# ThatRedox/ChunkyClPlugin

Hardware: AMD Instinct MI355X
Metric: Msamples/s, 32x32-chunk scene @1920x1080 (higher is better)
Workload: dtype f32

## Files before the change

### __graft_entry__.py

```python
import os
import sys

ROOT = os.path.dirname(os.path.abspath(__file__))
if ROOT not in sys.path:
    sys.path.insert(0, ROOT)


def build() -> None:
    from chunkyclplugin_amd import native
    path = native.build()
    native.build_tuning()
    lib = native.lib()
    missing = [s for s in native.declared_symbols() if not hasattr(lib, s)]
    if missing:
        raise RuntimeError(f"{path} does not export {missing}")
    from oracle import binding
    binding.port()
    binding.ref()
    binding.port_libm()
    binding.ref_libm()
    import subprocess
    out = os.path.join(native.CSRC, "build", "ubench_gather.o")
    os.makedirs(os.path.dirname(out), exist_ok=True)
    proc = subprocess.run(["hipcc", "--offload-arch=gfx950", "-O3", "-c", os.path.join(ROOT, "tools", "ubench_gather.hip"), "-o", out],
                          capture_output=True, text=True)
    if proc.returncode != 0:
        raise RuntimeError("hipcc failed on tools/ubench_gather.hip:\n" + proc.stderr[-2000:])
    exe = os.path.join(native.CSRC, "build", "host_example")
    proc = subprocess.run(["g++", "-std=c++17", "-I" + os.path.join(ROOT, "include"), os.path.join(ROOT, "examples", "host_example.cpp"), "-o", exe,
                           "-L" + native.PKG_DIR, "-lchunky_hip", "-Wl,-rpath," + native.PKG_DIR, "-Wl,--allow-shlib-undefined"],
                          capture_output=True, text=True)
    if proc.returncode != 0:
        raise RuntimeError("g++ failed on examples/host_example.cpp:\n" + proc.stderr[-2000:])
    import chunkyclplugin_amd


def smoke() -> None:
    import numpy as np
    from chunkyclplugin_amd import scenes
    from chunkyclplugin_amd.renderer import HipPathTracingRenderer, HipSceneLoader, RendererInstance
    from oracle import binding

    sc = scenes.tiny_scene(width=96, height=64)
    seeds = scenes.java_random_ints(4)
    inst = RendererInstance.get(0)
    loader = HipSceneLoader(inst)
    loader.load_packed(sc)
    r = HipPathTracingRenderer(loader, sc.width, sc.height)
    r.set_camera(sc.projector_type, sc.camera)
    r.render_passes(seeds)
# ... 17 lines not shown
```

### chunkyclplugin_amd/csrc/capi_host.cpp

```cpp
#include "capi_host.hpp"

#include <cmath>
#include <cstring>
#include <mutex>

#include "../../include/chunky_hip.h"
#include "camera_proj.h"
#include "capi_error.hpp"
#include "rt_math.h"
#include "widetree.hpp"

using namespace chunky;

int check_ints(const int32_t* p, int64_t n, const char* what) {
    if (n < 0 || (n > 0 && !p)) return fail(CHUNKY_E_INVALID, "%s: bad array (n=%lld)", what, (long long)n);
    return CHUNKY_OK;
}

static_assert(RT_PROJ_PARALLEL == CHUNKY_PROJ_PARALLEL && RT_PROJ_FISHEYE == CHUNKY_PROJ_FISHEYE && RT_PROJ_PANORAMIC == CHUNKY_PROJ_PANORAMIC &&
                  RT_PROJ_PANORAMIC_SLOT == CHUNKY_PROJ_PANORAMIC_SLOT && RT_PROJ_STEREOGRAPHIC == CHUNKY_PROJ_STEREOGRAPHIC &&
                  RT_PROJ_ODS == CHUNKY_PROJ_ODS && RT_PROJ_ODS_STACKED == CHUNKY_PROJ_ODS_STACKED, "camera_proj.h");
bool is_projected_type(int type) {
    return (type >= CHUNKY_PROJ_PARALLEL && type <= CHUNKY_PROJ_STEREOGRAPHIC) || type == CHUNKY_PROJ_ODS || type == CHUNKY_PROJ_ODS_STACKED;
}
int check_projected(const char* who, int type, const float* s, int64_t n, int height) {
    if (!is_projected_type(type))
        return fail(CHUNKY_E_INVALID, "%s: projector type %d is not a projected camera (1-5, 7, 8)", who, type);
    if (!s) return fail(CHUNKY_E_INVALID, "%s: NULL settings", who);
    if (n != 15) return fail(CHUNKY_E_INVALID, "%s: projector type %d needs 15 floats, got %lld", who, type, (long long)n);
    for (int i = 0; i < 15; i++)
        if (!std::isfinite(s[i])) return fail(CHUNKY_E_INVALID, "%s: settings[%d] is not finite", who, i);
    if (s[12] != 0.0f) return fail(CHUNKY_E_INVALID, "%s: settings[12] must be 0 for projector type %d (its lens is set by chunky_render_set_lens)", who, type);
    if (!(s[14] > 0.0f)) return fail(CHUNKY_E_INVALID, "%s: settings[14] must be > 0, got %g", who, (double)s[14]);
    if (s[13] != 0.0f && (type == CHUNKY_PROJ_FISHEYE || type == CHUNKY_PROJ_PANORAMIC || type == CHUNKY_PROJ_STEREOGRAPHIC))
        return fail(CHUNKY_E_INVALID, "%s: settings[13] must be 0 for projector type %d", who, type);
    if (type == CHUNKY_PROJ_ODS_STACKED) {
        if (s[13] < 0.0f) return fail(CHUNKY_E_INVALID, "%s: the stacked ODS image needs an eye offset >= 0, got %g", who, (double)s[13]);
        if (height % 2 != 0) return fail(CHUNKY_E_INVALID, "%s: the stacked ODS image needs an even height, got %d", who, height);
// ... 102 lines not shown
```

### chunkyclplugin_amd/csrc/capi_scene.hip

```cpp
#include "capi_internal.hpp"

#ifndef CHUNKY_BVH_TOP_RECORDS
#define CHUNKY_BVH_TOP_RECORDS 0
#endif
#ifndef CHUNKY_BVH_TREELET_RECORDS
#define CHUNKY_BVH_TREELET_RECORDS 0
#endif
static void bvh_layout_params(int* top, int* treelet) {
    *top = CHUNKY_BVH_TOP_RECORDS;
    *treelet = CHUNKY_BVH_TREELET_RECORDS;
#ifdef CHUNKY_TUNING
    if (const char* e = getenv("CHUNKY_BVH_LAYOUT")) {
        int a = 0, b = 0;
        if (sscanf(e, "%d,%d", &a, &b) == 2 && a >= 0 && b >= 0) {
            *top = a;
            *treelet = b;
        }
    }
#endif
}

extern "C" int chunky_scene_create(chunky_ctx* ctx, chunky_scene** out) {
    if (!ctx || !out) return fail(CHUNKY_E_INVALID, "chunky_scene_create: NULL argument");
    std::unique_ptr<chunky_scene> s(new chunky_scene);
// ... 306 lines not shown
            s->tri_off = nodes.size() * 4;
            nodes.insert(nodes.end(), tris.begin(), tris.end());
            HIP_TRY(s->bvh_rec.upload(nodes.data(), nodes.size() * 4, s->ctx->stream));
        }
        s->bvh_dirty = false;
    }
    if (want_emitters)
        if (int rc = refresh_emitters(s)) return rc;
    v->emitters = want_emitters ? (const int4*)s->emitters.p : nullptr;
    v->n_emitters = want_emitters ? (int)(s->host_emitters.size() / 4) : 0;
    v->n_block_ints = (int)(s->host_blocks.size() < 0x7FFFFFFFu ? s->host_blocks.size() : 0x7FFFFFFFu);
    v->sort_blocks = s->model_leaf_permille >= kSortBlocksPermille ? 1 : 0;
    v->bvh_rec = (const int4*)s->bvh_rec.p;
    v->tri_rec = s->bvh_rec.p ? (const int4*)((const char*)s->bvh_rec.p + s->tri_off) : nullptr;
    v->tri_off = (unsigned)s->tri_off;
    v->world_root = s->world_root;
    v->actor_root = s->actor_root;
    v->quad_aux = (const float*)s->quad_aux.p;
    v->bvh_stack_entries = (s->world_height > s->actor_height ? s->world_height : s->actor_height) + 1;
    v->block_info = (const int4*)s->block_info.p;
    v->mat8 = (const int4*)s->mat8.p;
    v->aabb_rec = (const int4*)s->aabb_rec.p;
    v->quad_rec = (const int4*)s->quad_rec.p;
    v->wide = s->wide_meta.nlev > 0 ? (const uint32_t*)s->wide.p : nullptr;
    v->wide_nlev = s->wide_meta.nlev;
    for (int i = 0; i < 6; i++) {
        v->wide_shift[i] = s->wide_meta.shift[i];
        v->wide_bits[i] = s->wide_meta.bits[i];
    }
    return CHUNKY_OK;
}
```

### chunkyclplugin_amd/csrc/path_state.hpp

```cpp
#pragma once
#include <hip/hip_runtime.h>

#include "kernels.hpp"
#include "rt_device.hpp"

namespace chunky {

struct LdsStack {
    int* base;
    int stride;
    DEV void push(int slot, int v) { base[slot * stride] = v; }
    DEV int pop(int slot) { return base[slot * stride]; }
};
template <int TREE>
DEV void leaf_lookup(const SceneView& S, int bx, int by, int bz, int& data, int& level, int& kind, bool inside = true, int* entry = nullptr) {
    if (TREE < 16 && !inside) bx = by = bz = 0;
    if (TREE == 0) {
        const int* __restrict__ tree = S.octree;
        level = S.octree_depth;
        data = tree[0];
        while (data > 0) {
            level--;
            data = tree[data + ((((bx >> level) & 1) << 2) | (((by >> level) & 1) << 1) | ((bz >> level) & 1))];
        }
        data = -data;
        kind = (data == 0 || data == kAnyType || (unsigned)data + 1u >= (unsigned)S.n_block_ints) ? 2 : 1;
    } else {
        const uint32_t* __restrict__ tree = S.wide;
        int e = 0;
        if (TREE >= 16) {
            constexpr int N3 = TREE - 16;
            {
                const int tb = S.wide_bits[0];
                unsigned idx = (((((unsigned)bx >> (3 * N3)) << tb) | ((unsigned)by >> (3 * N3))) << tb) | ((unsigned)bz >> (3 * N3));
                idx = inside ? idx : 0u;
                e = *(const int*)((const char*)tree + (idx << 2));
            }
#pragma unroll
            for (int i = 0; i < N3; i++) {
                if (e >= 0) {
                    const int sh = 3 * (N3 - 1 - i);
                    const unsigned xs = sh <= 6 ? (unsigned)bx << (6 - sh) : (unsigned)bx >> (sh - 6);
                    const unsigned ys = sh <= 3 ? (unsigned)by << (3 - sh) : (unsigned)by >> (sh - 3);
                    unsigned idx = ((unsigned)bz >> sh) & 7u;
                    asm("v_and_or_b32 %0, %1, 56, %0" : "+v"(idx) : "v"(ys));
                    asm("v_and_or_b32 %0, %1, %2, %0" : "+v"(idx) : "v"(xs), "s"(0x1c0u));
                    e = *(const int*)((const char*)tree + (((unsigned)e + idx) << 2));
                }
            }
        } else
#pragma unroll
        for (int i = 0; i < 6; i++) {
            if (i < S.wide_nlev && e >= 0) {
                const int sh = S.wide_shift[i], b = S.wide_bits[i];
                const unsigned ix = __builtin_amdgcn_ubfe((unsigned)bx, sh, b), iy = __builtin_amdgcn_ubfe((unsigned)by, sh, b),
                               iz = __builtin_amdgcn_ubfe((unsigned)bz, sh, b);
                e = (int)tree[(unsigned)e + ((((ix << b) | iy) << b) | iz)];
            }
        }
        level = (e >> 26) & 15;
        kind = (unsigned)e >= 0xC0000000u ? 2 : 0;
        data = (int)((unsigned)e & 0x1FFFFFFu);
        if (entry) *entry = e;
    }
}

template <int TREE>
DEV bool octree_hit(const SceneView& S, f3 o, f3 d, int draw_depth, Hit& h) {
    const int depth = S.octree_depth;
    float dist_march = 0;
    f3 inv = rcp3(d);
// ... 555 lines not shown
```

### chunkyclplugin_amd/csrc/render_pool.hip

```cpp
#include <hip/hip_runtime.h>

#include <cstdlib>

#include "path_state.hpp"
#include "pool_walk.hpp"

#ifndef CHUNKY_STAGING_STORE
#define CHUNKY_STAGING_STORE 0
#endif

namespace chunky {

template <int TREE, bool BVH>
DEV int shade_phase_ext(const SceneView& S, const RenderOpts& O, LaneState& L) {
    const bool hit = BVH ? L.trace_hit : L.oct_hit;
    const int kind = L.tkind;
    const f3 n = L.h.normal;
    int next = 0;
    if (kind == 0) {
        if (!hit) {
            L.radiance = L.radiance + sky_radiance(S, L.d, L.throughput, 1.0f);
            return ST_NEXT;
        }
        const f3 d_in = L.d;
        L.o = L.o + L.d * (L.h.distance - kOffset);
// ... 503 lines not shown
    if (chosen) *chosen = KernelChoice{tree, 1, bvh ? 1 : 0, grid, park, ext ? 1 : 0, sorted_ran ? 1 : 0};
    e = hipMemsetAsync(work_counter, 0, sizeof(int), stream);
    if (e != hipSuccess) return e;
    e = hipMemsetAsync(work_counter + kXcdCounters, 0, kXcdRanges * sizeof(int), stream);
    if (e != hipSuccess) return e;
    const WaveArgs A = make_wave_args(S, C, O, T, P, work_counter, res, (unsigned long long*)(work_counter + 2), (unsigned)depth, staging, (unsigned)n_samples,
                                      (unsigned)((n_tiles + kXcdRanges - 1) / kXcdRanges * kSampleTile * P.n), fast_div((unsigned)P.n * (unsigned)kSubBlock),
                                      fast_div((unsigned)((C.width + kTileEdge - 1) >> kTileLog)), seeds_dev);
    hipLaunchKernelGGL(k, dim3(grid), dim3(block), lds, stream, A);
    e = hipGetLastError();
    if (e != hipSuccess) return e;
    if (fold_stats) {
        return launch_fold_stats(staging, res, fold_stats, T, C.width, C.height, n_tiles, P.n, P.first_spp, stream);
    }
    const long long threads = 3ll * n_tiles * kSampleTile;
    hipLaunchKernelGGL(fold_kernel, dim3((unsigned)((threads + 255) / 256)), dim3(256), 0, stream, (const float*)staging, res, T,
                       C.width * C.height, C.width, n_tiles * kSampleTile, P.n, P.first_spp);
    return hipGetLastError();
}
bool pool_kernel_applies(int variant, const SceneView& S, const RenderOpts& O, bool have_queue_and_staging) {
    const bool any_bvh = !S.world_bvh_empty || !S.actor_bvh_empty;
    const bool steps_fit = (any_bvh || opts_extended(O) || O.draw_depth <= 65535) && O.max_depth <= 254;
    const bool form0_fits = S.wide != nullptr || (!any_bvh && !opts_extended(O) && !(variant & 4));
    return !(variant & 2) && !(variant & 8) && have_queue_and_staging && steps_fit && form0_fits &&
           (!any_bvh || (S.bvh_rec && S.tri_rec && S.mat8 && !(variant & 1)));
}
hipError_t launch_render(int variant, const SceneView& S, const CameraView& C, const RenderOpts& O, const ShardView& T,
                         const PassSeeds& P, float* res, int* work_counter, hipStream_t stream, KernelChoice* chosen,
                         float* staging, const int* seeds_dev) {
    return launch_render_stats(variant, S, C, O, T, P, res, work_counter, stream, chosen, staging, seeds_dev, nullptr);
}
hipError_t launch_render_stats(int variant, const SceneView& S, const CameraView& C, const RenderOpts& O, const ShardView& T,
                               const PassSeeds& P, float* res, int* work_counter, hipStream_t stream, KernelChoice* chosen,
                               float* staging, const int* seeds_dev, float* fold_stats) {
    if (pool_kernel_applies(variant, S, O, work_counter && staging)) {
        if (P.n > kMaxPoolPasses || (P.n > kMaxPassesPerLaunch && !seeds_dev)) return hipErrorInvalidValue;
        return launch_pool(variant, S, C, O, T, P, res, work_counter, stream, chosen, staging, P.n > kMaxPassesPerLaunch ? seeds_dev : nullptr, fold_stats);
    }
    if (fold_stats) return hipErrorNotSupported;
    if (P.n > kMaxPassesPerLaunch) return hipErrorInvalidValue;
    if (T.world != 1 && T.tile == 0) {
        if (!T.list) return hipErrorNotSupported;
        ShardView F = T;
        F.n_local = T.n_list;
        return launch_fallback(variant, S, C, O, F, P, res, work_counter, stream, chosen);
    }
    return launch_fallback(variant, S, C, O, T, P, res, work_counter, stream, chosen);
// ... 22 lines not shown
```

### chunkyclplugin_amd/csrc/rt_device.hpp

```cpp
#pragma once
#include <hip/hip_runtime.h>
#include <stdint.h>

#include "rt_math.h"
#include "camera_proj.h"

namespace chunky {

constexpr float kEps = 0.000005f;
constexpr float kOffset = 0.0001f;
constexpr int kAnyType = 0x7FFFFFFE;

struct f3 {
    float x, y, z;
};
struct f4 {
    float x, y, z, w;
};
#define DEV __device__ __forceinline__

DEV f3 mk3(float x, float y, float z) { return f3{x, y, z}; }
DEV f3 operator+(f3 a, f3 b) { return f3{a.x + b.x, a.y + b.y, a.z + b.z}; }
DEV f3 operator-(f3 a, f3 b) { return f3{a.x - b.x, a.y - b.y, a.z - b.z}; }
DEV f3 operator*(f3 a, f3 b) { return f3{a.x * b.x, a.y * b.y, a.z * b.z}; }
DEV f3 operator*(f3 a, float s) { return f3{a.x * s, a.y * s, a.z * s}; }
DEV float dot(f3 a, f3 b) { return rt_dot3(a.x, a.y, a.z, b.x, b.y, b.z); }
DEV f3 cross(f3 a, f3 b) {
    return f3{rt_cross_c(a.y, b.z, a.z, b.y), rt_cross_c(a.z, b.x, a.x, b.z), rt_cross_c(a.x, b.y, a.y, b.x)};
// ... 10 lines not shown
    const int* __restrict__ octree;
    const int* __restrict__ blocks;
    const int* __restrict__ quads;
    const int* __restrict__ aabbs;
    const int* __restrict__ world_bvh;
    const int* __restrict__ actor_bvh;
    const int* __restrict__ trigs;
    const uint32_t* __restrict__ atlas;
    const int* __restrict__ materials;
    const float4* __restrict__ sky;
    int octree_depth;
    int atlas_w, atlas_h, atlas_layers;
    int sky_w, sky_h;
    float sky_intensity;
    int sun_flags, sun_tex_size, sun_tex;
    float sun_intensity;
    f3 su, sv, sw;
    float sun_radius_cos;
    int world_bvh_empty, actor_bvh_empty;
    int bvh_stack_entries;
    const uint32_t* __restrict__ wide;
    int wide_nlev;
    int wide_shift[6], wide_bits[6];
    const int4* __restrict__ block_info;
    int sort_blocks;
    int n_block_ints;
    const float* __restrict__ quad_aux;
    const int4* __restrict__ mat8;
    const int4* __restrict__ aabb_rec;
    const int4* __restrict__ quad_rec;
    const int4* __restrict__ bvh_rec;
    const int4* __restrict__ tri_rec;
    unsigned tri_off;
    int world_root, actor_root;
    const int4* __restrict__ emitters;
    int n_emitters;
    int bvh_cull;
};

struct CameraView {
    const float* __restrict__ rays;
    int projector_type;
    float pos[3], m[9];
    float aperture, subject_distance, fov_tan;
    int width, height;
    float half_width, inv_height;
// ... 38 lines not shown
    Slabs s = slabs(x0, x1, y0, y1, z0, z1, o, inv);
    float tn = slab_near(s), tf = slab_far(s);
    return (tf < tn) ? rt_nan() : tn;
}
DEV float box_quick_far(float x0, float x1, float y0, float y1, float z0, float z1, f3 o, f3 inv, float& tf) {
    Slabs s = slabs(x0, x1, y0, y1, z0, z1, o, inv);
    float tn = slab_near(s);
    tf = slab_far(s);
    return (tf < tn) ? rt_nan() : tn;
}
DEV float box_exit(float x0, float x1, float y0, float y1, float z0, float z1, f3 o, f3 inv) {
    return slab_far(slabs(x0, x1, y0, y1, z0, z1, o, inv));
}

DEV f4 color_from_argb(unsigned argb) {
    const float k = 1.0f / 256.0f;
    return f4{(float)((argb >> 16) & 0xFF) * k, (float)((argb >> 8) & 0xFF) * k, (float)(argb & 0xFF) * k,
              (float)((argb >> 24) & 0xFF) * k};
}
DEV f4 unpack_unorm8(uint32_t t) {
    return f4{rt_unorm8(t & 0xFF), rt_unorm8((t >> 8) & 0xFF), rt_unorm8((t >> 16) & 0xFF), rt_unorm8(t >> 24)};
}

DEV uint32_t atlas_texel(const SceneView& S, float u, float v, int location, int size) {
    int width = (size >> 16) & 0xFFFF, height = size & 0xFFFF;
    v = 1 - v;
    int x = rt_clampi((int)((u - kEps) * (float)width), 0, width - 1);
    int y = rt_clampi((int)((v - kEps) * (float)height), 0, height - 1);
    x += ((location >> 22) & 0x1FF) * 16;
    y += ((location >> 13) & 0x1FF) * 16;
    int d = location & 0x7FFFF;
    x = rt_clampi(x, 0, S.atlas_w - 1);
    y = rt_clampi(y, 0, S.atlas_h - 1);
    d = rt_clampi(d, 0, S.atlas_layers - 1);
    return S.atlas[((size_t)d * S.atlas_h + y) * S.atlas_w + x];
}

__device__ __constant__ const float kEmittanceLut[256] = {
#include "emit_lut.inc"
};

DEV bool material_eval(const SceneView& S, unsigned flags, unsigned tint, unsigned tex_size, unsigned color_w,
                       unsigned ne, float u, float v, Hit& h, int m5 = 0);
DEV bool material_sample(const SceneView& S, int material, float u, float v, Hit& h) {
    const int* m = S.materials + material;
    return material_eval(S, m[0], m[1], m[2], m[3], m[4], u, v, h, m[5]);
}
DEV bool material_eval(const SceneView& S, unsigned flags, unsigned tint, unsigned tex_size, unsigned color_w,
                       unsigned ne, float u, float v, Hit& h, int m5) {
    f4 c = (flags & 4) ? unpack_unorm8(atlas_texel(S, u, v, (int)color_w, (int)tex_size)) : color_from_argb(color_w);
    if (!(c.w > kEps)) return false;
    unsigned tt = tint >> 24;
    if (tt == 0xFF || tt == 1 || tt == 2 || tt == 3) {
        unsigned tc = tt == 0xFF ? tint : (tt == 1 ? 0xFF71A74Du : (tt == 2 ? 0xFF8EB971u : 0xFF3F76E4u));
        f4 t = color_from_argb(tc);
        c = f4{c.x * t.x, c.y * t.y, c.z * t.z, c.w * t.w};
    }
// ... 107 lines not shown
        float u = dot(pt, xv) / xx;
        float v = dot(pt, yv) / yy;
        if (!(u >= 0 && u <= 1 && v >= 0 && v <= 1)) continue;
        float tu = as_float(q[9]) + (u * as_float(q[10]));
        float tv = as_float(q[11]) + (v * as_float(q[12]));
        if (material_sample(S, q[13], tu, tv, h)) {
            h.normal = n;
            best = t;
            hit = true;
        }
    }
    return hit ? best : rt_nan();
}

DEV bool material_sample8(const SceneView& S, int m8, float u, float v, Hit& h) {
    const int4 a = S.mat8[m8], b = S.mat8[m8 + 1];
    return material_eval(S, a.x, a.y, a.z, a.w, b.x, u, v, h, b.y);
}

DEV float aabb_model_hit_rec(const SceneView& S, int rec, f3 no, f3 dir, f3 inv, Hit& h) {
    const int boxes = rec & 0xFF, first = (int)((unsigned)rec >> 8);
    float best = rt_inf();
    bool hit = false;
    for (int i = 0; i < boxes; i++) {
        const int4 r0 = S.aabb_rec[(first + i) * 3], r1 = S.aabb_rec[(first + i) * 3 + 1], r2 = S.aabb_rec[(first + i) * 3 + 2];
        Slabs s = slabs(as_float(r0.x), as_float(r0.y), as_float(r0.z), as_float(r0.w), as_float(r1.x), as_float(r1.y), no, inv);
        float tn = slab_near(s), tf = slab_far(s);
        if (tf < tn) continue;
        if (tn != tn || tn >= best || tn < -kEps) continue;
        Face f = face_map2(s, tn, no + dir * tn);
        const int fl_all = r1.z;
        int mat = r1.w, fl = 0;
        if (f.n.x == 1) { mat = r1.w; fl = fl_all >> 4; }
        if (f.n.z == -1) { mat = r2.x; fl = fl_all >> 8; }
        if (f.n.x == -1) { mat = r2.y; fl = fl_all >> 12; }
        if (f.n.y == 1) { mat = r2.z; fl = fl_all >> 16; }
        if (f.n.y == -1) { mat = r2.w; fl = fl_all >> 20; }
        if (fl & 8) continue;
        float u = f.u, v = f.v;
        if (fl & 4) u = 1 - u;
        if (fl & 2) v = 1 - v;
        if (fl & 1) { float t = u; u = v; v = t; }
        if (material_sample8(S, mat, u, v, h)) {
            h.normal = f.n;
            best = tn;
            hit = true;
        }
    }
    return hit ? best : rt_nan();
}

DEV float quad_model_hit_rec(const SceneView& S, int rec, f3 no, f3 dir, Hit& h) {
    const int quads = rec & 0xFF, first = (int)((unsigned)rec >> 8);
    float best = rt_inf();
    bool hit = false;
    for (int i = 0; i < quads; i++) {
        const int4* __restrict__ q = S.quad_rec + (first + i) * 6;
        const int4 r0 = q[0], r1 = q[1], r2 = q[2], r4 = q[4];
        const f3 qo = mk3(as_float(r0.x), as_float(r0.y), as_float(r0.z));
        const f3 xv = mk3(as_float(r1.x), as_float(r1.y), as_float(r1.z));
        const f3 yv = mk3(as_float(r2.x), as_float(r2.y), as_float(r2.z));
        const f3 n = mk3(as_float(r4.x), as_float(r4.y), as_float(r4.z));
        const float n_qo = as_float(r0.w), xx = as_float(r1.w), yy = as_float(r2.w);
        float denom = dot(dir, n);
        if (!(denom < -kEps)) continue;
        float t = -(dot(no, n) - n_qo) / denom;
        if (!(t > -kEps && t < best)) continue;
        f3 pt = (no + dir * t) - qo;
        float u = dot(pt, xv) / xx;
        float v = dot(pt, yv) / yy;
        if (!(u >= 0 && u <= 1 && v >= 0 && v <= 1)) continue;
        const int4 r3 = q[3], r5 = q[5];
        float tu = as_float(r3.x) + (u * as_float(r3.y));
        float tv = as_float(r3.z) + (v * as_float(r3.w));
        if (material_eval(S, r5.x, r5.y, r5.z, r5.w, r4.w, tu, tv, h, (int)((unsigned)r4.w >> 8))) {
            h.normal = n;
            best = t;
            hit = true;
        }
    }
    return hit ? best : rt_nan();
}

enum : int { kBlockAny = 0, kBlockCubes = 1, kBlockModels = 2 };
template <int KINDS = kBlockAny>
DEV float block_hit(const SceneView& S, int block, int bx, int by, int bz, f3 pos, f3 dir, f3 inv, Hit& h) {
    if (KINDS == kBlockAny && block == kAnyType) return rt_nan();
    f3 no = (pos - dir * kOffset) - mk3((float)bx, (float)by, (float)bz);
    int type, ptr;
    if (KINDS != kBlockAny || S.block_info) {
        const int4 a = S.block_info[(unsigned)block], b = S.block_info[(unsigned)block + 1u];
        type = a.x;
        ptr = a.y;
        if (KINDS != kBlockModels && type == 1) return cube_hit(S, a.z, a.w, b.x, b.y, b.z, no, pos, inv, h, b.w);
        if (KINDS == kBlockCubes) return rt_nan();
// ... 99 lines not shown
                stack.push(to_visit++, cur + 7);
                cur = second;
            }
        }
    }
    return hit;
}

struct SkyTexels {
    float4 t00, t10, t01, t11;
    float a, b;
};
constexpr float kSkyTwoPi = RT_PI_F * 2;
constexpr float kSunDiscRadius = 0.03f, kSunDiscWidth = kSunDiscRadius * 4, kSunDiscWidth2 = kSunDiscWidth * 2;
DEV SkyTexels sky_fetch(const SceneView& S, f3 d) {
    float theta = rt_atan2(d.z, d.x);
    theta = rt_div_const(theta, kSkyTwoPi);
    theta = rt_fmod1(rt_fmod1(theta) + 1);
    float phi = (rt_asin(rt_clamp(d.y, -1.0f, 1.0f)) + RT_PI_2_F) * RT_1_PI_F;
    int i0, i1, j0, j1;
    SkyTexels k;
    rt_mirror_linear(theta, S.sky_w, &i0, &i1, &k.a);
    rt_mirror_linear(phi, S.sky_h, &j0, &j1, &k.b);
    k.t00 = S.sky[j0 * S.sky_w + i0];
    k.t10 = S.sky[j0 * S.sky_w + i1];
    k.t01 = S.sky[j1 * S.sky_w + i0];
    k.t11 = S.sky[j1 * S.sky_w + i1];
    return k;
}
DEV f4 sky_blend(const SceneView& S, const SkyTexels& q) {
    const float a = q.a, b = q.b;
    float w00 = (1.0f - a) * (1.0f - b), w10 = a * (1.0f - b), w01 = (1.0f - a) * b, w11 = a * b;
    float k = S.sky_intensity;
    return f4{(w00 * q.t00.x + w10 * q.t10.x + w01 * q.t01.x + w11 * q.t11.x) * k,
              (w00 * q.t00.y + w10 * q.t10.y + w01 * q.t01.y + w11 * q.t11.y) * k,
              (w00 * q.t00.z + w10 * q.t10.z + w01 * q.t01.z + w11 * q.t11.z) * k, 0.0f};
}
DEV f4 sky_color(const SceneView& S, f3 d) { return sky_blend(S, sky_fetch(S, d)); }

DEV void sun_disc(const SceneView& S, f3 d, f4& c) {
    if (!(S.sun_flags & 1) || dot(d, S.sw) < 0.5f) return;
    const float width = kSunDiscWidth, width2 = kSunDiscWidth2;
    float a = RT_PI_2_F - rt_acos(dot(d, S.su)) + width;
    if (a >= 0 && a < width2) {
        float b = RT_PI_2_F - rt_acos(dot(d, S.sv)) + width;
        if (b >= 0 && b < width2) {
// ... 136 lines not shown
```

### chunkyclplugin_amd/csrc/scene_records.cpp

```cpp
#include "scene_records.hpp"

#include <algorithm>
#include <cstddef>
#include <utility>

#include "rt_math.h"

namespace chunky {

bool build_quad_aux(const std::vector<int32_t>& B, const std::vector<int32_t>& Q, std::vector<float>* out) {
    out->assign(Q.size(), 0.0f);
    std::vector<int64_t> owner(Q.size(), -1);
    bool any = false;
    for (size_t k = 0; k + 1 < B.size(); k += 2) {
        if (B[k] != 3) continue;
        const int64_t ptr = B[k + 1];
        if (ptr < 0 || (size_t)ptr >= Q.size()) return false;
        const int64_t count = Q[(size_t)ptr];
        if (count < 0 || (size_t)(ptr + 1 + 15 * count) > Q.size()) return false;
        for (int64_t i = 0; i < count; i++) {
            const int64_t q = ptr + 1 + 15 * i;
            for (int w = 0; w < 6; w++) {
                if (owner[(size_t)(q + w)] >= 0 && owner[(size_t)(q + w)] != q) return false;
                owner[(size_t)(q + w)] = q;
// ... 8 lines not shown
            a[0] = nx;
            a[1] = ny;
            a[2] = nz;
            a[3] = rt_dot3(nx, ny, nz, f[0], f[1], f[2]);
            a[4] = rt_dot3(f[3], f[4], f[5], f[3], f[4], f[5]);
            a[5] = rt_dot3(f[6], f[7], f[8], f[6], f[7], f[8]);
            any = true;
        }
    }
    return any;
}

int model_leaf_permille(const std::vector<int32_t>& T, const std::vector<int32_t>& B) {
    int64_t cubes = 0, models = 0;
    for (const int32_t v : T) {
        if (v > 0) continue;
        const int64_t ptr = -(int64_t)v;
        if (ptr == 0 || ptr + 1 >= (int64_t)B.size()) continue;
        const int32_t type = B[(size_t)ptr];
        cubes += type == 1;
        models += type == 2 || type == 3;
    }
    return cubes + models > 0 ? (int)(models * 1000 / (cubes + models)) : 0;
}

void derive_records(const std::vector<int32_t>& B, const std::vector<int32_t>& M, const std::vector<int32_t>& A, const std::vector<int32_t>& Q,
                    DerivedRecords* out) {
    const size_t n_blocks = B.size() / 2, n_mats = M.size() / 6;
    std::vector<int32_t>&mat8 = out->mat8, &info = out->info, &aabb_rec = out->aabb_rec, &quad_rec = out->quad_rec;
    mat8.assign(n_mats * 8, 0);
    for (size_t m = 0; m < n_mats; m++)
        for (int w = 0; w < 6; w++) mat8[m * 8 + w] = M[m * 6 + w];
    auto mat_index = [&](int32_t ptr, int32_t* out) {
        if (ptr < 0 || ptr % 6 != 0 || (size_t)ptr / 6 >= n_mats) return false;
        *out = (ptr / 6) * 2;
        return true;
    };
    info.assign(n_blocks * 8, 0);
    aabb_rec.clear();
    quad_rec.clear();
    std::vector<int64_t> aabb_at(A.size(), -1), quad_at(Q.size(), -1);
    for (size_t k = 0; k < n_blocks; k++) {
        int32_t* e = &info[k * 8];
        const int32_t type = B[2 * k], ptr = B[2 * k + 1];
        e[0] = type;
        e[1] = ptr;
// ... 318 lines not shown
```

### chunkyclplugin_amd/csrc/scene_records.hpp

```cpp
#pragma once
#include <cstdint>
#include <cstring>
#include <vector>

namespace chunky {

inline float bits_to_float(int32_t i) {
    float f;
    memcpy(&f, &i, 4);
    return f;
}

constexpr int kSortBlocksPermille = 30;
int model_leaf_permille(const std::vector<int32_t>& octree, const std::vector<int32_t>& blocks);

struct DerivedRecords {
    std::vector<int32_t> info, mat8, aabb_rec, quad_rec;
};
void derive_records(const std::vector<int32_t>& blocks, const std::vector<int32_t>& materials, const std::vector<int32_t>& aabbs,
                    const std::vector<int32_t>& quads, DerivedRecords* out);

bool build_quad_aux(const std::vector<int32_t>& blocks, const std::vector<int32_t>& quads, std::vector<float>* out);

bool bvh_links_height(const std::vector<int32_t>& nodes, int* height);

bool bvh_leaves_sound(const std::vector<int32_t>& nodes, bool empty, const std::vector<int32_t>& trigs, const std::vector<int32_t>& materials);

bool build_bvh_records(const std::vector<int32_t>& world_nodes, bool world_empty, const std::vector<int32_t>& actor_nodes, bool actor_empty,
                       const std::vector<int32_t>& trigs, const std::vector<int32_t>& materials, int top, int treelet,
                       std::vector<int32_t>* bvh_rec, std::vector<int32_t>* tri_rec, int* world_root, int* actor_root);

void list_emitters(const std::vector<int32_t>& octree, int depth, const std::vector<int32_t>& blocks, const std::vector<int32_t>& materials,
                   std::vector<int32_t>* out);

}
```

### chunkyclplugin_amd/native.py

```python
from __future__ import annotations

import ctypes as C
import os
import re
import subprocess
from typing import List, Optional

import numpy as np

PKG_DIR = os.path.dirname(os.path.abspath(__file__))
CSRC = os.path.join(PKG_DIR, "csrc")
LIB_PATH = os.environ.get("CHUNKY_HIP_LIB") or os.path.join(PKG_DIR, "libchunky_hip.so")
HEADER = os.path.join(os.path.dirname(PKG_DIR), "include", "chunky_hip.h")
SOURCES = ["render_pool.hip", "render_pool_bvh.hip", "render_fallback.hip", "aux_kernels.hip", "filter.hip", "aov.hip", "denoise.hip", "adaptive.hip",
           "capi_context.hip", "capi_group.hip", "capi_scene.hip", "capi_render.hip", "capi_aov.hip", "capi_adaptive.hip", "capi_denoise.hip",
           "capi_run.hip", "capi_filter.hip", "capi_selftest.hip", "capi_error.cpp", "capi_host.cpp", "adaptive_host.cpp", "denoise_host.cpp",
           "scene_records.cpp", "widetree.cpp"]
HIPCC_FLAGS = ["--offload-arch=gfx950", "-O3", "-std=c++17", "-ffp-contract=off", "-fno-slp-vectorize", "-fPIC", "-shared"]

MAX_TRACES = 10
HIT_DTYPE = np.dtype([("hit", "<i4"), ("material", "<i4"), ("distance", "<f4"), ("normal", "<f4", 3),
                      ("color", "<f4", 4), ("emittance", "<f4"), ("point", "<f4", 3)])

PALETTE_BLOCK, PALETTE_MATERIAL, PALETTE_AABB, PALETTE_QUAD, PALETTE_TRIG = range(5)
# ... 188 lines not shown
            "chunky_render_adaptive_kernel_time": [vp, C.POINTER(f32), C.POINTER(C.c_int)],
            "chunky_selftest_render_list": [vp, vp, C.c_int, vp, C.c_int],
            "chunky_adaptive_host_begin": [C.c_int, C.c_int, C.POINTER(AdaptiveParams), C.POINTER(AdaptiveState), vp, vp, vp, vp],
            "chunky_adaptive_host_resume": [C.POINTER(AdaptiveState), vp, C.c_int, vp, vp, vp, vp],
            "chunky_adaptive_state_check": [C.POINTER(AdaptiveState), vp, vp],
            "chunky_render_adaptive_ex": [vp, vp, C.c_int, C.POINTER(AdaptiveParams), C.POINTER(AdaptiveCallbacks), C.POINTER(AdaptiveSummary)],
            "chunky_render_adaptive_resume": [vp, vp, C.c_int, C.POINTER(AdaptiveParams), C.POINTER(AdaptiveCallbacks), C.POINTER(AdaptiveSummary)],
            "chunky_render_adaptive_state": [vp, C.POINTER(AdaptiveState), vp, i64],
            "chunky_render_adaptive_restore": [vp, C.POINTER(AdaptiveState), vp, vp, vp, vp],
            "chunky_render_run": [vp, vp, C.POINTER(i32), i32, i32, POST_RENDER_FN, vp],
            "chunky_render_run_ex": [vp, vp, C.POINTER(i32), i32, i32, C.POINTER(RunCallbacks)],
            "chunky_java_random_ints": [i64, vp, C.c_int],
            "chunky_selftest_math": [vp, C.c_int, C.c_int, vp, vp, vp],
            "chunky_selftest_helpers": [vp, C.c_int, C.c_int, C.c_int, vp, vp, C.POINTER(i32)],
            "chunky_selftest_gamma_scan": [vp, C.c_int, C.c_uint32, C.c_uint64, C.POINTER(C.c_uint64), C.POINTER(f32)],
            "chunky_selftest_camera_rays": [vp, i32, vp, i64],
            "chunky_selftest_shard_map": [vp, C.c_int, C.c_int, C.c_int, C.c_int, C.c_int, C.c_int, C.c_int, vp, vp, vp],
            "chunky_camera_rays": [C.c_int, vp, i64, C.c_int, C.c_int, i32, vp],
            "chunky_camera_rays_lens": [C.c_int, vp, i64, C.c_int, C.c_int, i32, f32, f32, vp],
            "chunky_filter_frame": [vp, C.c_int, C.c_int, C.c_double, vp, vp, C.c_int],
            "chunky_filter_gamma_thresholds": [vp],
            "chunky_filter_frame_device": [vp, i64, f32, vp, vp, C.c_int, C.c_int, C.POINTER(f32)],
            "chunky_widetree_lookup": [vp, i64, C.c_int, vp, C.c_int, vp, C.c_int, vp, vp, C.POINTER(i64)],
        }
        for name, args in sig.items():
            if not hasattr(L, name) and os.environ.get("CHUNKY_HIP_LIB") and os.environ.get("CHUNKY_HIP_LIB_EARLIER") == "1":
                continue
            fn = getattr(L, name)
            fn.argtypes = args
            fn.restype = C.c_int
        _lib = L
    return _lib


def check(rc: int) -> None:
    if rc != 0:
        raise ChunkyHipError(rc, (lib().chunky_last_error() or b"").decode("utf-8", "replace"))


def ptr(a: np.ndarray) -> int:
    return a.ctypes.data


def java_random_ints(n: int, seed: int = 0) -> np.ndarray:
    out = np.zeros(n, np.int32)
    check(lib().chunky_java_random_ints(seed, ptr(out), n))
# ... 2 lines not shown

def camera_rays(projector_type: int, settings, width: int, height: int, seed: int, lens=None) -> np.ndarray:
    s = np.ascontiguousarray(settings, np.float32)
    out = np.zeros(int(width) * int(height) * 6, np.float32)
    seed32 = int(np.int32(np.uint32(seed & 0xFFFFFFFF)))
    if lens is None:
        check(lib().chunky_camera_rays(int(projector_type), ptr(s), s.size, int(width), int(height), seed32, ptr(out)))
    else:
        check(lib().chunky_camera_rays_lens(int(projector_type), ptr(s), s.size, int(width), int(height), seed32, float(lens[0]), float(lens[1]), ptr(out)))
    return out


def widetree_lookup(tree: np.ndarray, depth: int, xyz: np.ndarray, level_bits=None):
    tree = np.ascontiguousarray(tree, np.int32)
    xyz = np.ascontiguousarray(xyz, np.int32).reshape(-1, 3)
    data = np.zeros(len(xyz), np.int32)
    level = np.zeros(len(xyz), np.int32)
    n_entries = C.c_int64()
    lb = None if level_bits is None else np.ascontiguousarray(level_bits, np.int32)
    check(lib().chunky_widetree_lookup(ptr(tree), tree.size, depth, None if lb is None else ptr(lb),
                                       0 if lb is None else lb.size, ptr(xyz), len(xyz), ptr(data), ptr(level),
                                       C.byref(n_entries)))
    return data, level, n_entries.value


def denoise_params(iterations: Optional[int] = None, sigma_color: Optional[float] = None, sigma_normal: Optional[float] = None,
                   sigma_albedo: Optional[float] = None, demodulate: Optional[bool] = None, kernel: int = 0) -> DenoiseParams:
    p = DenoiseParams()
    check(lib().chunky_denoise_default_params(C.byref(p)))
    if iterations is not None:
        p.iterations = int(iterations)
    if sigma_color is not None:
        p.sigma_color = float(sigma_color)
    if sigma_normal is not None:
        p.sigma_normal = float(sigma_normal)
    if sigma_albedo is not None:
        p.sigma_albedo = float(sigma_albedo)
    if demodulate is not None:
        p.flags = (p.flags & ~DENOISE_DEMODULATE) | (DENOISE_DEMODULATE if demodulate else 0)
    p.flags |= int(kernel) << DENOISE_KERNEL_SHIFT
    return p


def _images(width, height, *arrays):
    out = []
    for a in arrays:
# ... 102 lines not shown
```

### chunkyclplugin_amd/renderer.py

```python
from __future__ import annotations

import ctypes as C
import struct
from typing import Callable, Optional

import numpy as np

from . import native
from .native import check, ptr


def camera_rays(projector_type: int, settings, width: int, height: int, seed: int, lens=None) -> np.ndarray:
    return native.camera_rays(projector_type, settings, width, height, seed, lens)


def denoise_frame(instance, width: int, height: int, color, albedo, normal, params=None) -> np.ndarray:
    c, a, n = native._images(width, height, color, albedo, normal)
    p = params if params is not None else native.denoise_params()
    out = np.empty((int(height), int(width), 3), np.float32)
    check(native.lib().chunky_denoise_frame(instance._h, int(width), int(height), ptr(c), ptr(a), ptr(n), C.byref(p), ptr(out)))
    return out


class RendererInstance:
# ... 103 lines not shown
                          (native.PALETTE_TRIG, sc.bvh_trigs)):
            a = i32(arr)
            check(L.chunky_scene_set_palette(self._h, kind, ptr(a), a.size))
        for which, arr in ((native.BVH_WORLD, sc.world_bvh), (native.BVH_ACTOR, sc.actor_bvh)):
            a = i32(arr)
            check(L.chunky_scene_set_bvh(self._h, which, ptr(a), a.size))
        atlas = np.ascontiguousarray(sc.atlas, np.uint8)
        layers, h, w, _ = atlas.shape
        check(L.chunky_scene_set_atlas(self._h, ptr(atlas), w, h, layers))
        sky = np.ascontiguousarray(sc.sky, np.uint8)
        check(L.chunky_scene_set_sky(self._h, ptr(sky), sky.shape[1], sky.shape[0], float(sc.sky_intensity)))
        sun = i32(sc.sun)
        check(L.chunky_scene_set_sun(self._h, ptr(sun)))
        self.packed = sc
        return True

    def emitters(self) -> np.ndarray:
        n = C.c_int32()
        check(native.lib().chunky_scene_emitters(self._h, None, 0, C.byref(n)))
        out = np.zeros((max(n.value, 1), 4), np.int32)
        check(native.lib().chunky_scene_emitters(self._h, ptr(out), n.value, C.byref(n)))
        return out[:n.value]

    def selftest_helpers(self, which: int, rows, tree: int = 1):
        rows = np.ascontiguousarray(rows, np.float32).reshape(-1, 32)
        out = np.zeros((len(rows), 12), np.float32)
        used = C.c_int32()
        check(native.lib().chunky_selftest_helpers(self._h, which, tree, len(rows), ptr(rows), ptr(out), C.byref(used)))
        return out, used.value

    def load_octree(self, tree_data, depth: int, block_mapping) -> None:
        t = np.ascontiguousarray(tree_data, np.int32)
        m = np.ascontiguousarray(block_mapping, np.int32)
        check(native.lib().chunky_scene_load_octree(self._h, ptr(t), t.size, depth, ptr(m), m.size))

    def close(self) -> None:
        if self._h:
            check(native.lib().chunky_scene_destroy(self._h))
            self._h = C.c_void_p()


class HipPathTracingRenderer:

    ID = "ChunkyClRenderer"

    def __init__(self, scene_loader: HipSceneLoader, width: int, height: int):
# ... 291 lines not shown
```

### include/chunky_hip.h

```cpp
#ifndef CHUNKY_HIP_H
#define CHUNKY_HIP_H

#include <stddef.h>
#include <stdint.h>

#ifdef __cplusplus
extern "C" {
#endif

typedef enum chunky_status {
    CHUNKY_OK = 0,
    CHUNKY_E_INVALID = -1,
    CHUNKY_E_NO_DEVICE = -2,
    CHUNKY_E_HIP = -3,
    CHUNKY_E_STATE = -4,
    CHUNKY_E_ABORTED = -5
} chunky_status;

typedef struct chunky_ctx chunky_ctx;
typedef struct chunky_scene chunky_scene;
typedef struct chunky_render chunky_render;

int chunky_device_count(void);
int chunky_device_name(int device, char* buf, int buf_len);
// ... 202 lines not shown
    void (*merged)(void* user, int32_t sample_spp);
    int (*save_event)(void* user, int32_t spp);
    void (*regenerate_camera)(void* user);
    void* user;
    int (*poll_gate)(void* user);
} chunky_run_callbacks;
int chunky_render_run_ex(chunky_render* r, double* sample_buffer, int32_t* scene_spp, int32_t target_spp,
                         int32_t merge_interval, const chunky_run_callbacks* callbacks);
int chunky_java_random_ints(int64_t seed, int32_t* out, int n);

#define CHUNKY_FILTER_GAMMA 0
#define CHUNKY_FILTER_TONEMAP1 1
#define CHUNKY_FILTER_ACES 2
#define CHUNKY_FILTER_HABLE 3
int chunky_filter_frame(chunky_ctx* ctx, int width, int height, double exposure, const double* input,
                        int32_t* argb_out, int type);
int chunky_filter_gamma_thresholds(float* out256);
int chunky_filter_frame_device(chunky_ctx* ctx, int64_t n_pixels, float exposure, const void* d_input, void* d_argb,
                               int type, int repeat, float* kernel_ms);

int chunky_widetree_lookup(const int32_t* tree, int64_t n_ints, int depth, const int32_t* level_bits, int n_levels,
                           const int32_t* xyz , int n, int32_t* data_out, int32_t* level_out, int64_t* n_entries);

int chunky_selftest_math(chunky_ctx* ctx, int which, int n, const float* a, const float* b, float* out);

int chunky_selftest_helpers(chunky_scene* scene, int which, int tree, int n, const float* in_rows, float* out_rows, int32_t* tree_used);

int chunky_selftest_camera_rays(chunky_render* r, int32_t seed, float* out, int64_t n_floats);

int chunky_selftest_shard_map(chunky_ctx* ctx, int mode, int width, int height, int rank, int world, int tile, int n,
                              const uint32_t* pairs, int32_t* out, int32_t view_out[4]);

int chunky_selftest_gamma_scan(chunky_ctx* ctx, int curve, uint32_t first_bits, uint64_t count, uint64_t* mismatches, float* worst_estimate);

#ifdef __cplusplus
}
#endif
#endif
```

Baseline: 8123.

## Use 32-bit offset addressing for atlas, sky and record loads in pool kernel

Adds a per-scene addr32 capability word, computed on the host from atlas, sky and record buffer sizes. When every form fits, the pool render kernel computes texel, sky and AABB/quad record addresses with 32-bit offsets and v_mad_u32_u24 instead of 64-bit index arithmetic, which is meant to cut VALU work and VGPR pressure. It also hoists the octree-march index computation out of the e>=0 branch so the address math runs unconditionally. Scenes whose bounds do not fit now fail the pool kernel's eligibility check and take another path.

```diff
diff --git a/__graft_entry__.py b/__graft_entry__.py
--- a/__graft_entry__.py
+++ b/__graft_entry__.py
@@ -20,12 +20,13 @@
     binding.port_libm()
     binding.ref_libm()
     import subprocess
-    out = os.path.join(native.CSRC, "build", "ubench_gather.o")
-    os.makedirs(os.path.dirname(out), exist_ok=True)
-    proc = subprocess.run(["hipcc", "--offload-arch=gfx950", "-O3", "-c", os.path.join(ROOT, "tools", "ubench_gather.hip"), "-o", out],
-                          capture_output=True, text=True)
-    if proc.returncode != 0:
-        raise RuntimeError("hipcc failed on tools/ubench_gather.hip:\n" + proc.stderr[-2000:])
+    for tool in ("ubench_gather", "ubench_imul"):
+        out = os.path.join(native.CSRC, "build", tool + ".o")
+        os.makedirs(os.path.dirname(out), exist_ok=True)
+        proc = subprocess.run(["hipcc", "--offload-arch=gfx950", "-O3", "-c", os.path.join(ROOT, "tools", tool + ".hip"), "-o", out],
+                              capture_output=True, text=True)
+        if proc.returncode != 0:
+            raise RuntimeError(f"hipcc failed on tools/{tool}.hip:\n" + proc.stderr[-2000:])
     exe = os.path.join(native.CSRC, "build", "host_example")
     proc = subprocess.run(["g++", "-std=c++17", "-I" + os.path.join(ROOT, "include"), os.path.join(ROOT, "examples", "host_example.cpp"), "-o", exe,
                            "-L" + native.PKG_DIR, "-lchunky_hip", "-Wl,-rpath," + native.PKG_DIR, "-Wl,--allow-shlib-undefined"],
diff --git a/chunkyclplugin_amd/csrc/addr32.h b/chunkyclplugin_amd/csrc/addr32.h
--- /dev/null
+++ b/chunkyclplugin_amd/csrc/addr32.h
@@ -0,0 +1,11 @@
+#pragma once
+
+namespace chunky {
+
+enum : unsigned {
+    kAddr32Atlas = 1,
+    kAddr32Sky = 2,
+    kAddr32Records = 4,
+};
+
+}
diff --git a/chunkyclplugin_amd/csrc/capi_host.cpp b/chunkyclplugin_amd/csrc/capi_host.cpp
--- a/chunkyclplugin_amd/csrc/capi_host.cpp
+++ b/chunkyclplugin_amd/csrc/capi_host.cpp
@@ -8,12 +8,23 @@
 #include "camera_proj.h"
 #include "capi_error.hpp"
 #include "rt_math.h"
+#include "scene_records.hpp"
 #include "widetree.hpp"
 
 using namespace chunky;
 
 int check_ints(const int32_t* p, int64_t n, const char* what) {
     if (n < 0 || (n > 0 && !p)) return fail(CHUNKY_E_INVALID, "%s: bad array (n=%lld)", what, (long long)n);
+    return CHUNKY_OK;
+}
+
+extern "C" int chunky_addr32_word(const int64_t dims[5], const uint64_t bytes[2], int indices_checked, uint32_t* word) {
+    if (!dims || !bytes || !word) return fail(CHUNKY_E_INVALID, "addr32_word: NULL");
+    AddrBounds b;
+    b.atlas_w = dims[0], b.atlas_h = dims[1], b.atlas_layers = dims[2], b.sky_w = dims[3], b.sky_h = dims[4];
+    b.aabb_rec_bytes = bytes[0], b.quad_rec_bytes = bytes[1];
+    b.indices_checked = indices_checked != 0;
+    *word = addr32_word(b);
     return CHUNKY_OK;
 }
 
diff --git a/chunkyclplugin_amd/csrc/capi_scene.hip b/chunkyclplugin_amd/csrc/capi_scene.hip
--- a/chunkyclplugin_amd/csrc/capi_scene.hip
+++ b/chunkyclplugin_amd/csrc/capi_scene.hip
@@ -352,6 +352,16 @@
     v->mat8 = (const int4*)s->mat8.p;
     v->aabb_rec = (const int4*)s->aabb_rec.p;
     v->quad_rec = (const int4*)s->quad_rec.p;
+    {
+        AddrBounds b;
+        b.atlas_w = s->atlas_w, b.atlas_h = s->atlas_h, b.atlas_layers = s->atlas_layers, b.sky_w = s->sky_w, b.sky_h = s->sky_h;
+        b.aabb_rec_bytes = s->aabb_rec.bytes, b.quad_rec_bytes = s->quad_rec.bytes;
+        b.indices_checked = !s->derived_dirty && s->block_info.p != nullptr;
+        v->addr32 = addr32_word(b);
+#ifdef CHUNKY_TUNING
+        if (const char* e = getenv("CHUNKY_ADDR32_MASK")) v->addr32 &= (unsigned)atoi(e);
+#endif
+    }
     v->wide = s->wide_meta.nlev > 0 ? (const uint32_t*)s->wide.p : nullptr;
     v->wide_nlev = s->wide_meta.nlev;
     for (int i = 0; i < 6; i++) {
@@ -360,3 +370,13 @@
     }
     return CHUNKY_OK;
 }
+
+extern "C" int chunky_scene_addr32(chunky_scene* scene, uint32_t* word) {
+    if (scene && !scene->replicas.empty()) return chunky_scene_addr32(scene->replicas[0], word);
+    LOCK_SCENE(scene);
+    if (!word) return fail(CHUNKY_E_INVALID, "scene_addr32: NULL");
+    SceneView v;
+    if (int rc = scene_view(scene, &v, false)) return rc;
+    *word = v.addr32;
+    return CHUNKY_OK;
+}
diff --git a/chunkyclplugin_amd/csrc/path_state.hpp b/chunkyclplugin_amd/csrc/path_state.hpp
--- a/chunkyclplugin_amd/csrc/path_state.hpp
+++ b/chunkyclplugin_amd/csrc/path_state.hpp
@@ -38,6 +38,16 @@
             }
 #pragma unroll
             for (int i = 0; i < N3; i++) {
+#if defined(CHUNKY_MARCH_HOIST) && CHUNKY_MARCH_HOIST
+                const int sh = 3 * (N3 - 1 - i);
+                const unsigned xs = sh <= 6 ? (unsigned)bx << (6 - sh) : (unsigned)bx >> (sh - 6);
+                const unsigned ys = sh <= 3 ? (unsigned)by << (3 - sh) : (unsigned)by >> (sh - 3);
+                unsigned idx = ((unsigned)bz >> sh) & 7u;
+                asm("v_and_or_b32 %0, %1, 56, %0" : "+v"(idx) : "v"(ys));
+                asm("v_and_or_b32 %0, %1, %2, %0" : "+v"(idx) : "v"(xs), "s"(0x1c0u));
+                asm volatile("" : "+v"(idx));
+                if (e >= 0) e = *(const int*)((const char*)tree + (((unsigned)e + idx) << 2));
+#else
                 if (e >= 0) {
                     const int sh = 3 * (N3 - 1 - i);
                     const unsigned xs = sh <= 6 ? (unsigned)bx << (6 - sh) : (unsigned)bx >> (sh - 6);
@@ -47,6 +57,7 @@
                     asm("v_and_or_b32 %0, %1, %2, %0" : "+v"(idx) : "v"(xs), "s"(0x1c0u));
                     e = *(const int*)((const char*)tree + (((unsigned)e + idx) << 2));
                 }
+#endif
             }
         } else
 #pragma unroll
diff --git a/chunkyclplugin_amd/csrc/render_pool.hip b/chunkyclplugin_amd/csrc/render_pool.hip
--- a/chunkyclplugin_amd/csrc/render_pool.hip
+++ b/chunkyclplugin_amd/csrc/render_pool.hip
@@ -1,6 +1,13 @@
 #include <hip/hip_runtime.h>
 
 #include <cstdlib>
+
+#if !defined(CHUNKY_POOL_BVH_TU) && !defined(CHUNKY_ADDR32_FORMS)
+#define CHUNKY_ADDR32_FORMS 7
+#endif
+#if !defined(CHUNKY_POOL_BVH_TU) && !defined(CHUNKY_MARCH_HOIST)
+#define CHUNKY_MARCH_HOIST 1
+#endif
 
 #include "path_state.hpp"
 #include "pool_walk.hpp"
@@ -550,7 +557,8 @@
     const bool any_bvh = !S.world_bvh_empty || !S.actor_bvh_empty;
     const bool steps_fit = (any_bvh || opts_extended(O) || O.draw_depth <= 65535) && O.max_depth <= 254;
     const bool form0_fits = S.wide != nullptr || (!any_bvh && !opts_extended(O) && !(variant & 4));
-    return !(variant & 2) && !(variant & 8) && have_queue_and_staging && steps_fit && form0_fits &&
+    const bool addr_fits = any_bvh || (S.addr32 & (unsigned)(CHUNKY_ADDR32_FORMS)) == (unsigned)(CHUNKY_ADDR32_FORMS);
+    return !(variant & 2) && !(variant & 8) && have_queue_and_staging && steps_fit && form0_fits && addr_fits &&
            (!any_bvh || (S.bvh_rec && S.tri_rec && S.mat8 && !(variant & 1)));
 }
 hipError_t launch_render(int variant, const SceneView& S, const CameraView& C, const RenderOpts& O, const ShardView& T,
diff --git a/chunkyclplugin_amd/csrc/rt_device.hpp b/chunkyclplugin_amd/csrc/rt_device.hpp
--- a/chunkyclplugin_amd/csrc/rt_device.hpp
+++ b/chunkyclplugin_amd/csrc/rt_device.hpp
@@ -4,6 +4,7 @@
 
 #include "rt_math.h"
 #include "camera_proj.h"
+#include "addr32.h"
 
 namespace chunky {
 
@@ -60,6 +61,7 @@
     const uint32_t* __restrict__ wide;
     int wide_nlev;
     int wide_shift[6], wide_bits[6];
+    unsigned addr32;
     const int4* __restrict__ block_info;
     int sort_blocks;
     int n_block_ints;
@@ -144,6 +146,20 @@
     return f4{rt_unorm8(t & 0xFF), rt_unorm8((t >> 8) & 0xFF), rt_unorm8((t >> 16) & 0xFF), rt_unorm8(t >> 24)};
 }
 
+#ifndef CHUNKY_ADDR32_FORMS
+#define CHUNKY_ADDR32_FORMS 0
+#endif
+#define CHUNKY_ADDR32(bit) (((CHUNKY_ADDR32_FORMS) & (bit)) != 0)
+template <typename T>
+DEV T load_at(const void* __restrict__ base, unsigned byte_offset) {
+    return *(const T*)((const char*)base + byte_offset);
+}
+DEV unsigned mad_u24(unsigned a, unsigned b_uniform, unsigned c) {
+    unsigned r;
+    asm("v_mad_u32_u24 %0, %1, %2, %3" : "=v"(r) : "v"(a), "s"(b_uniform), "v"(c));
+    return r;
+}
+
 DEV uint32_t atlas_texel(const SceneView& S, float u, float v, int location, int size) {
     int width = (size >> 16) & 0xFFFF, height = size & 0xFFFF;
     v = 1 - v;
@@ -155,6 +171,8 @@
     x = rt_clampi(x, 0, S.atlas_w - 1);
     y = rt_clampi(y, 0, S.atlas_h - 1);
     d = rt_clampi(d, 0, S.atlas_layers - 1);
+    if (CHUNKY_ADDR32(kAddr32Atlas))
+        return load_at<uint32_t>(S.atlas, mad_u24(mad_u24((unsigned)d, (unsigned)S.atlas_h, (unsigned)y), (unsigned)S.atlas_w, (unsigned)x) << 2);
     return S.atlas[((size_t)d * S.atlas_h + y) * S.atlas_w + x];
 }
 
@@ -308,8 +326,14 @@
     const int boxes = rec & 0xFF, first = (int)((unsigned)rec >> 8);
     float best = rt_inf();
     bool hit = false;
-    for (int i = 0; i < boxes; i++) {
-        const int4 r0 = S.aabb_rec[(first + i) * 3], r1 = S.aabb_rec[(first + i) * 3 + 1], r2 = S.aabb_rec[(first + i) * 3 + 2];
+    unsigned off = (unsigned)first * 48u;
+    for (int i = 0; i < boxes; i++, off += 48u) {
+        int4 r0, r1, r2;
+        if (CHUNKY_ADDR32(kAddr32Records)) {
+            r0 = load_at<int4>(S.aabb_rec, off), r1 = load_at<int4>(S.aabb_rec, off + 16u), r2 = load_at<int4>(S.aabb_rec, off + 32u);
+        } else {
+            r0 = S.aabb_rec[(first + i) * 3], r1 = S.aabb_rec[(first + i) * 3 + 1], r2 = S.aabb_rec[(first + i) * 3 + 2];
+        }
         Slabs s = slabs(as_float(r0.x), as_float(r0.y), as_float(r0.z), as_float(r0.w), as_float(r1.x), as_float(r1.y), no, inv);
         float tn = slab_near(s), tf = slab_far(s);
         if (tf < tn) continue;
@@ -340,9 +364,17 @@
     const int quads = rec & 0xFF, first = (int)((unsigned)rec >> 8);
     float best = rt_inf();
     bool hit = false;
-    for (int i = 0; i < quads; i++) {
+    constexpr bool a32 = CHUNKY_ADDR32(kAddr32Records);
+    unsigned off = (unsigned)first * 96u;
+    for (int i = 0; i < quads; i++, off += 96u) {
         const int4* __restrict__ q = S.quad_rec + (first + i) * 6;
-        const int4 r0 = q[0], r1 = q[1], r2 = q[2], r4 = q[4];
+        int4 r0, r1, r2, r4;
+        if (a32) {
+            r0 = load_at<int4>(S.quad_rec, off), r1 = load_at<int4>(S.quad_rec, off + 16u), r2 = load_at<int4>(S.quad_rec, off + 32u),
+            r4 = load_at<int4>(S.quad_rec, off + 64u);
+        } else {
+            r0 = q[0], r1 = q[1], r2 = q[2], r4 = q[4];
+        }
         const f3 qo = mk3(as_float(r0.x), as_float(r0.y), as_float(r0.z));
         const f3 xv = mk3(as_float(r1.x), as_float(r1.y), as_float(r1.z));
         const f3 yv = mk3(as_float(r2.x), as_float(r2.y), as_float(r2.z));
@@ -356,7 +388,12 @@
         float u = dot(pt, xv) / xx;
         float v = dot(pt, yv) / yy;
         if (!(u >= 0 && u <= 1 && v >= 0 && v <= 1)) continue;
-        const int4 r3 = q[3], r5 = q[5];
+        int4 r3, r5;
+        if (a32) {
+            r3 = load_at<int4>(S.quad_rec, off + 48u), r5 = load_at<int4>(S.quad_rec, off + 80u);
+        } else {
+            r3 = q[3], r5 = q[5];
+        }
         float tu = as_float(r3.x) + (u * as_float(r3.y));
         float tv = as_float(r3.z) + (v * as_float(r3.w));
         if (material_eval(S, r5.x, r5.y, r5.z, r5.w, r4.w, tu, tv, h, (int)((unsigned)r4.w >> 8))) {
@@ -502,6 +539,14 @@
     SkyTexels k;
     rt_mirror_linear(theta, S.sky_w, &i0, &i1, &k.a);
     rt_mirror_linear(phi, S.sky_h, &j0, &j1, &k.b);
+    if (CHUNKY_ADDR32(kAddr32Sky)) {
+        const unsigned pitch = (unsigned)S.sky_w << 4, c0 = (unsigned)i0 << 4, c1 = (unsigned)i1 << 4;
+        k.t00 = load_at<float4>(S.sky, mad_u24((unsigned)j0, pitch, c0));
+        k.t10 = load_at<float4>(S.sky, mad_u24((unsigned)j0, pitch, c1));
+        k.t01 = load_at<float4>(S.sky, mad_u24((unsigned)j1, pitch, c0));
+        k.t11 = load_at<float4>(S.sky, mad_u24((unsigned)j1, pitch, c1));
+        return k;
+    }
     k.t00 = S.sky[j0 * S.sky_w + i0];
     k.t10 = S.sky[j0 * S.sky_w + i1];
     k.t01 = S.sky[j1 * S.sky_w + i0];
diff --git a/chunkyclplugin_amd/csrc/scene_records.cpp b/chunkyclplugin_amd/csrc/scene_records.cpp
--- a/chunkyclplugin_amd/csrc/scene_records.cpp
+++ b/chunkyclplugin_amd/csrc/scene_records.cpp
@@ -54,6 +54,18 @@
         models += type == 2 || type == 3;
     }
     return cubes + models > 0 ? (int)(models * 1000 / (cubes + models)) : 0;
+}
+
+unsigned addr32_word(const AddrBounds& b) {
+    constexpr int64_t k24 = (int64_t)1 << 24;
+    constexpr uint64_t k32 = (uint64_t)1 << 32;
+    unsigned word = 0;
+    if (b.atlas_w > 0 && b.atlas_h > 0 && b.atlas_layers > 0 && b.atlas_w < k24 && b.atlas_h < k24 && b.atlas_layers < k24 &&
+        b.atlas_layers * b.atlas_h < k24 && (uint64_t)(b.atlas_layers * b.atlas_h) * (uint64_t)b.atlas_w * 4 < k32)
+        word |= kAddr32Atlas;
+    if (b.sky_w > 0 && b.sky_h > 0 && b.sky_w * 16 < k24 && b.sky_h < k24 && (uint64_t)b.sky_w * (uint64_t)b.sky_h * 16 < k32) word |= kAddr32Sky;
+    if (b.indices_checked && b.aabb_rec_bytes < k32 && b.quad_rec_bytes < k32) word |= kAddr32Records;
+    return word;
 }
 
 void derive_records(const std::vector<int32_t>& B, const std::vector<int32_t>& M, const std::vector<int32_t>& A, const std::vector<int32_t>& Q,
diff --git a/chunkyclplugin_amd/csrc/scene_records.hpp b/chunkyclplugin_amd/csrc/scene_records.hpp
--- a/chunkyclplugin_amd/csrc/scene_records.hpp
+++ b/chunkyclplugin_amd/csrc/scene_records.hpp
@@ -2,6 +2,8 @@
 #include <cstdint>
 #include <cstring>
 #include <vector>
+
+#include "addr32.h"
 
 namespace chunky {
 
@@ -20,6 +22,13 @@
 void derive_records(const std::vector<int32_t>& blocks, const std::vector<int32_t>& materials, const std::vector<int32_t>& aabbs,
                     const std::vector<int32_t>& quads, DerivedRecords* out);
 
+struct AddrBounds {
+    int64_t atlas_w = 0, atlas_h = 0, atlas_layers = 0, sky_w = 0, sky_h = 0;
+    uint64_t aabb_rec_bytes = 0, quad_rec_bytes = 0;
+    bool indices_checked = false;
+};
+unsigned addr32_word(const AddrBounds& b);
+
 bool build_quad_aux(const std::vector<int32_t>& blocks, const std::vector<int32_t>& quads, std::vector<float>* out);
 
 bool bvh_links_height(const std::vector<int32_t>& nodes, int* height);
diff --git a/chunkyclplugin_amd/native.py b/chunkyclplugin_amd/native.py
--- a/chunkyclplugin_amd/native.py
+++ b/chunkyclplugin_amd/native.py
@@ -234,6 +234,8 @@
             "chunky_filter_gamma_thresholds": [vp],
             "chunky_filter_frame_device": [vp, i64, f32, vp, vp, C.c_int, C.c_int, C.POINTER(f32)],
             "chunky_widetree_lookup": [vp, i64, C.c_int, vp, C.c_int, vp, C.c_int, vp, vp, C.POINTER(i64)],
+            "chunky_addr32_word": [vp, vp, C.c_int, C.POINTER(C.c_uint32)],
+            "chunky_scene_addr32": [vp, C.POINTER(C.c_uint32)],
         }
         for name, args in sig.items():
             if not hasattr(L, name) and os.environ.get("CHUNKY_HIP_LIB") and os.environ.get("CHUNKY_HIP_LIB_EARLIER") == "1":
@@ -282,6 +284,18 @@
                                        0 if lb is None else lb.size, ptr(xyz), len(xyz), ptr(data), ptr(level),
                                        C.byref(n_entries)))
     return data, level, n_entries.value
+
+
+ADDR32_ATLAS, ADDR32_SKY, ADDR32_RECORDS = 1, 2, 4
+
+
+def addr32_word(atlas=(1, 1, 1), sky=(1, 1), record_bytes=(0, 0), indices_checked: bool = True) -> int:
+    dims = np.array([*atlas, *sky], np.int64)
+    sizes = np.array(record_bytes, np.uint64)
+    assert dims.size == 5 and sizes.size == 2
+    word = C.c_uint32()
+    check(lib().chunky_addr32_word(ptr(dims), ptr(sizes), 1 if indices_checked else 0, C.byref(word)))
+    return word.value
 
 
 def denoise_params(iterations: Optional[int] = None, sigma_color: Optional[float] = None, sigma_normal: Optional[float] = None,
diff --git a/chunkyclplugin_amd/renderer.py b/chunkyclplugin_amd/renderer.py
--- a/chunkyclplugin_amd/renderer.py
+++ b/chunkyclplugin_amd/renderer.py
@@ -149,6 +149,11 @@
         check(native.lib().chunky_scene_emitters(self._h, ptr(out), n.value, C.byref(n)))
         return out[:n.value]
 
+    def addr32(self) -> int:
+        word = C.c_uint32()
+        check(native.lib().chunky_scene_addr32(self._h, C.byref(word)))
+        return word.value
+
     def selftest_helpers(self, which: int, rows, tree: int = 1):
         rows = np.ascontiguousarray(rows, np.float32).reshape(-1, 32)
         out = np.zeros((len(rows), 12), np.float32)
diff --git a/include/chunky_hip.h b/include/chunky_hip.h
--- a/include/chunky_hip.h
+++ b/include/chunky_hip.h
@@ -248,6 +248,9 @@
 int chunky_widetree_lookup(const int32_t* tree, int64_t n_ints, int depth, const int32_t* level_bits, int n_levels,
                            const int32_t* xyz , int n, int32_t* data_out, int32_t* level_out, int64_t* n_entries);
 
+int chunky_addr32_word(const int64_t dims[5], const uint64_t bytes[2], int indices_checked, uint32_t* word);
+int chunky_scene_addr32(chunky_scene* scene, uint32_t* word);
+
 int chunky_selftest_math(chunky_ctx* ctx, int which, int n, const float* a, const float* b, float* out);
 
 int chunky_selftest_helpers(chunky_scene* scene, int which, int tree, int n, const float* in_rows, float* out_rows, int32_t* tree_used);
```

After: 8267, median of 6. 1.8% higher.
